# XuyangBai/D3Feat

Hardware: NVIDIA H100
Metric: points/sec through KPFCNN encoder (higher is better)
Workload: dtype f32

## Files before the change

### d3feat_b200/csrc/neighbors.cu

```cuda
#include <stdlib.h>

#include "ops.cuh"
#include "sort.cuh"

namespace d3f {

struct NbGrid {
  float minx, miny, minz, inv_cell;
  int nx, ny, nz;
  long long ncells;
};

static NbGrid make_grid(const float* host_bbox, float radius) {
  NbGrid g;
  float cell = radius * 1.001f;
  g.inv_cell = 1.0f / cell;
  g.minx = host_bbox[0];
  g.miny = host_bbox[1];
  g.minz = host_bbox[2];
  auto dim = [&](int a) {
    double ext = (double)host_bbox[3 + a] - (double)host_bbox[a];
    if (!(ext >= 0)) ext = 0;
    double n = floor(ext / (double)cell) + 2.0;
    return n > 2.0e9 ? 2000000000 : (int)n;
  };
  g.nx = dim(0);
  g.ny = dim(1);
  g.nz = dim(2);
  g.ncells = (long long)g.nx * g.ny * g.nz;
  return g;
}

constexpr long long kMaxGridCells = 1ll << 27;

__device__ __forceinline__ int cell_coord(float v, float mn, float inv, int n) {
  int c = (int)floorf((v - mn) * inv);
  return min(max(c, 0), n - 1);
}

__global__ void __launch_bounds__(256)
cell_count_kernel(const float* __restrict__ s, int Ns_cap, const int* __restrict__ ns_dev,
                  const int* __restrict__ start, int B, NbGrid g, uint32_t* __restrict__ cell_id,
                  int* __restrict__ cell_cnt) {
  const int Ns = dyn_rows(Ns_cap, ns_dev);
  int i = blockIdx.x * blockDim.x + threadIdx.x;
  if (i >= Ns) return;
  int b = batch_of(start, B, i);
  int cx = cell_coord(s[3 * (size_t)i], g.minx, g.inv_cell, g.nx);
  int cy = cell_coord(s[3 * (size_t)i + 1], g.miny, g.inv_cell, g.ny);
  int cz = cell_coord(s[3 * (size_t)i + 2], g.minz, g.inv_cell, g.nz);
  uint32_t c = (uint32_t)((long long)b * g.ncells + ((long long)cz * g.ny + cy) * g.nx + cx);
  cell_id[i] = c;
  atomicAdd(&cell_cnt[c], 1);
}

__global__ void __launch_bounds__(256)
cell_scatter_kernel(const float* __restrict__ s, int Ns_cap, const int* __restrict__ ns_dev,
                    const uint32_t* __restrict__ cell_id, const int* __restrict__ cell_start,
                    int* __restrict__ cell_cnt, float4* __restrict__ sorted_pts) {
  const int Ns = dyn_rows(Ns_cap, ns_dev);
  int i = blockIdx.x * blockDim.x + threadIdx.x;
  if (i >= Ns) return;
  uint32_t c = cell_id[i];
  int pos = cell_start[c] + atomicSub(&cell_cnt[c], 1) - 1;
  sorted_pts[pos] = make_float4(s[3 * (size_t)i], s[3 * (size_t)i + 1], s[3 * (size_t)i + 2], __uint_as_float((uint32_t)i));
}

__global__ void __launch_bounds__(256)
cell_order_kernel(const float4* __restrict__ sorted_pts, int Ns, int* __restrict__ out) {
  int i = blockIdx.x * blockDim.x + threadIdx.x;
  if (i < Ns) out[i] = (int)__float_as_uint(sorted_pts[i].w);
}

struct NbWs {
  uint32_t* cell_id;
  int* s_start;
  int* q_start;
  float4* sorted_pts;
  int* cell_start;
  int* cell_cnt;
  int* scan_scratch;
};

static size_t carve_nb(Carver& cv, int Ns, int B, long long total_cells, NbWs& w) {
  int n = Ns > 0 ? Ns : 1;
  w.cell_id = cv.take<uint32_t>(n);
  w.s_start = cv.take<int>(B + 1);
  w.q_start = cv.take<int>(B + 1);
  w.sorted_pts = cv.take<float4>(n);
  w.cell_start = cv.take<int>((size_t)total_cells + 1);
  w.cell_cnt = cv.take<int>((size_t)total_cells + 1);
  w.scan_scratch = cv.take<int>((size_t)scan_num_blocks((int)total_cells) + 1);
  return cv.off;
}

size_t radius_neighbors_workspace_bytes(int Ns, int B, float radius, const float* host_bbox) {
  if (host_bbox == nullptr || !(radius > 0.f) || B < 1) return 0;
  NbGrid g = make_grid(host_bbox, radius);
  long long total = g.ncells * B;
  if (total > kMaxGridCells) return 0;
  Carver cv(nullptr, ~(size_t)0);
  NbWs w;
  return carve_nb(cv, Ns, B, total, w) + 256;
}

int radius_neighbors_build(const float* supports, const int* s_batch_len, int B, int Ns, float radius,
                           const float* host_bbox, void* workspace, size_t workspace_bytes, cudaStream_t stream,
                           const int* ns_dev, const int* s_start_pre) {
  D3F_REQUIRE(B >= 1 && B <= kMaxBatch, D3F_ERR_INVALID, "radius_neighbors: B=%d must be in [1,%d]", B, kMaxBatch);
  D3F_REQUIRE(radius > 0.f && Ns >= 0 && host_bbox != nullptr, D3F_ERR_INVALID,
              "radius_neighbors: radius=%g Ns=%d invalid or host_bbox missing", (double)radius, Ns);
  NbGrid g = make_grid(host_bbox, radius);
  long long total = g.ncells * B;
  D3F_REQUIRE(total <= kMaxGridCells, D3F_ERR_CAPACITY,
              "radius_neighbors: grid %d x %d x %d x %d clouds exceeds %lld cells", g.nx, g.ny, g.nz, B,
              kMaxGridCells);
  D3F_REQUIRE(workspace_bytes >= radius_neighbors_workspace_bytes(Ns, B, radius, host_bbox), D3F_ERR_WORKSPACE,
              "radius_neighbors: workspace too small");
  Carver cv(workspace, workspace_bytes);
  NbWs w;
  carve_nb(cv, Ns, B, total, w);
  if (s_start_pre != nullptr) w.s_start = const_cast<int*>(s_start_pre);
  else if (launch_batch_start(s_batch_len, B, w.s_start, stream)) return D3F_ERR_CUDA;
  D3F_CUDA(cudaMemsetAsync(w.cell_cnt, 0, sizeof(int) * ((size_t)total + 1), stream));
  if (Ns == 0) {
    D3F_CUDA(cudaMemsetAsync(w.cell_start, 0, sizeof(int) * ((size_t)total + 1), stream));
    return D3F_OK;
  }
  cell_count_kernel<<<ceil_div(Ns, 256), 256, 0, stream>>>(supports, Ns, ns_dev, w.s_start, B, g, w.cell_id, w.cell_cnt);
  D3F_LAUNCH_CHECK("cell_count_kernel");
  if (exclusive_scan_i32(w.cell_cnt, w.cell_start, (int)total, w.cell_start + total, w.scan_scratch, stream))
    return D3F_ERR_CUDA;
  cell_scatter_kernel<<<ceil_div(Ns, 256), 256, 0, stream>>>(supports, Ns, ns_dev, w.cell_id, w.cell_start, w.cell_cnt,
                                                             w.sorted_pts);
  D3F_LAUNCH_CHECK("cell_scatter_kernel");
  return D3F_OK;
}

int radius_neighbors_order(const void* workspace, int Ns, int B, float radius, const float* host_bbox, int* out_order,
                           cudaStream_t stream) {
  D3F_REQUIRE(B >= 1 && radius > 0.f && host_bbox != nullptr, D3F_ERR_INVALID, "radius_neighbors_order: bad arguments");
  if (Ns <= 0) return D3F_OK;
  NbGrid g = make_grid(host_bbox, radius);
  long long total = g.ncells * B;
  D3F_REQUIRE(total <= kMaxGridCells, D3F_ERR_CAPACITY, "radius_neighbors: grid too large");
  Carver cv(const_cast<void*>(workspace), ~(size_t)0);
  NbWs w;
  carve_nb(cv, Ns, B, total, w);
  cell_order_kernel<<<ceil_div(Ns, 256), 256, 0, stream>>>(w.sorted_pts, Ns, out_order);
  D3F_LAUNCH_CHECK("cell_order_kernel");
  return D3F_OK;
}

constexpr int kNbWarps = 8;
constexpr int kNbListCap = 512;

struct Hit {
  float d2;
  int idx;
};

__device__ __forceinline__ bool hit_less(float da, int ia, float db, int ib) {
  return da < db || (da == db && ia < ib);
}

__device__ __forceinline__ float sq_dist_rn(float qx, float qy, float qz, float4 s) {
  float dx = __fsub_rn(qx, s.x), dy = __fsub_rn(qy, s.y), dz = __fsub_rn(qz, s.z);
  float r = __fmul_rn(dx, dx);
  r = __fadd_rn(r, __fmul_rn(dy, dy));
  r = __fadd_rn(r, __fmul_rn(dz, dz));
  return r;
}

template <int K>
__device__ __forceinline__ void bitonic_block2(unsigned& ka, unsigned& kb, int lane) {
  const bool asc = K == 64 || (lane & (K >> 1)) == 0;
#pragma unroll
  for (int j = K >> 1; j >= 2; j >>= 1) {
    const unsigned oa = __shfl_xor_sync(0xffffffffu, ka, j >> 1), ob = __shfl_xor_sync(0xffffffffu, kb, j >> 1);
    const bool keep_min = ((lane & (j >> 1)) == 0) == asc;
    ka = keep_min ? min(ka, oa) : max(ka, oa);
    kb = keep_min ? min(kb, ob) : max(kb, ob);
  }
  const unsigned lo = min(ka, kb), hi = max(ka, kb);
  ka = asc ? lo : hi;
  kb = asc ? hi : lo;
}

template <bool FILL>
__global__ void __launch_bounds__(kNbWarps * 32)
radius_query_kernel(const float* __restrict__ q, int Nq_cap, const int* __restrict__ nq_dev,
                    const int* __restrict__ q_start, int B, NbGrid g, const float4* __restrict__ sorted_pts,
                    const int* __restrict__ cell_start, float r2, int cols, int pad_value_in,
                    const int* __restrict__ pad_dev, int* __restrict__ counts, int* __restrict__ out_max,
                    int* __restrict__ out_idx) {
  const int Nq = dyn_rows(Nq_cap, nq_dev);
  const int pad_value = pad_dev ? __ldg(pad_dev) : pad_value_in;
  __shared__ int2 run_tab[kNbWarps][10];
  __shared__ Hit list[FILL ? kNbWarps : 1][FILL ? kNbListCap : 1];
  const int lane = threadIdx.x & 31, warp = threadIdx.x >> 5;
  const int qi = blockIdx.x * kNbWarps + warp;
  if (qi >= Nq) return;
  const float qx = q[3 * (size_t)qi], qy = q[3 * (size_t)qi + 1], qz = q[3 * (size_t)qi + 2];
  int b;
  if (B <= 32) {
    const bool le = lane < B && __ldg(q_start + lane) <= qi;
    b = max(__popc(__ballot_sync(0xffffffffu, le)) - 1, 0);
  } else {
    b = batch_of(q_start, B, qi);
  }
  const int cx = cell_coord(qx, g.minx, g.inv_cell, g.nx);
  const int cy = cell_coord(qy, g.miny, g.inv_cell, g.ny);
  const int cz = cell_coord(qz, g.minz, g.inv_cell, g.nz);

  int rs = 0, rl = 0;
  if (lane < 9) {
    const int dz = (lane * 11) >> 5;
    const int yy = cy + (lane - 3 * dz) - 1, zz = cz + dz - 1;
    if (yy >= 0 && yy < g.ny && zz >= 0 && zz < g.nz) {
      const int row = b * (int)g.ncells + (zz * g.ny + yy) * g.nx;
      const int x0 = max(cx - 1, 0), x1 = min(cx + 1, g.nx - 1);
      const int s = __ldg(cell_start + row + x0), e = __ldg(cell_start + row + x1 + 1);
      if (e > s) {
        rs = s;
        rl = e - s;
      }
    }
  }
  int inc = rl;
#pragma unroll
  for (int o = 1; o < 16; o <<= 1) {
    int t = __shfl_up_sync(0xffffffffu, inc, o);
    if (lane >= o) inc += t;
  }
  if (lane < 9) run_tab[warp][lane] = make_int2(inc, rs - (inc - rl));
  const int T = __shfl_sync(0xffffffffu, inc, 8);
  if (lane == 9) run_tab[warp][9] = make_int2(0x7fffffff, 0);
  __syncwarp();

  int n = 0;
  const int2* tp = &run_tab[warp][0];
  int2 cur = *tp;
  const unsigned below = (1u << lane) - 1u;
  for (int t0 = 0; t0 < T; t0 += 32) {
    const int t = t0 + lane;
    bool hit = false;
    float d2 = 0.f;
    int sidx = 0;
    if (t < T) {
      while (t >= cur.x) cur = *++tp;
      const float4 sp = __ldg(sorted_pts + (t + cur.y));
      d2 = sq_dist_rn(qx, qy, qz, sp);
      sidx = (int)__float_as_uint(sp.w);
      hit = d2 < r2;
    }
    const unsigned m = __ballot_sync(0xffffffffu, hit);
    if (FILL) {
      const int pos = n + __popc(m & below);
      if (hit && pos < kNbListCap) {
        list[warp][pos].d2 = d2;
        list[warp][pos].idx = sidx;
      }
    }
    n += __popc(m);
  }

  if (!FILL) {
    if (lane == 0) {
      counts[qi] = n;
      atomicMax(out_max, n);
    }
    return;
  }
  if (counts != nullptr && lane == 0) counts[qi] = n;
  if (out_max != nullptr && lane == 0) atomicMax(out_max, n);
  __syncwarp();
  int* row = out_idx + (size_t)qi * cols;
  bool sorted_fast = false;
  if (n <= 64) {
    const int ia = 2 * lane, ib = ia + 1;
    unsigned ka = 0xffffffffu, kb = 0xffffffffu;
    if (ia < n) ka = (__float_as_uint(list[warp][ia].d2) & ~63u) | (unsigned)ia;
    if (ib < n) kb = (__float_as_uint(list[warp][ib].d2) & ~63u) | (unsigned)ib;
    const int kmax = n <= 2 ? 2 : 2 << (31 - __clz(n - 1));
    if (kmax >= 2) bitonic_block2<2>(ka, kb, lane);
    if (kmax >= 4) bitonic_block2<4>(ka, kb, lane);
    if (kmax >= 8) bitonic_block2<8>(ka, kb, lane);
    if (kmax >= 16) bitonic_block2<16>(ka, kb, lane);
    if (kmax >= 32) bitonic_block2<32>(ka, kb, lane);
    if (kmax >= 64) bitonic_block2<64>(ka, kb, lane);
    const unsigned next_a = __shfl_down_sync(0xffffffffu, ka, 1);
    const bool clash = (ib < n && ((ka ^ kb) < 64u)) || (ib + 1 < n && lane < 31 && ((kb ^ next_a) < 64u));
    if (!__any_sync(0xffffffffu, clash)) {
      if (ia < n && ia < cols) row[ia] = list[warp][ka & 63u].idx;
      if (ib < n && ib < cols) row[ib] = list[warp][kb & 63u].idx;
      sorted_fast = true;
    }
  }
  if (sorted_fast) {
  } else if (n <= 64) {
    const unsigned long long kInf = ~0ull;
    unsigned long long a = kInf, b = kInf;
    if (lane < n) a = ((unsigned long long)__float_as_uint(list[warp][lane].d2) << 32) | (unsigned)list[warp][lane].idx;
    if (n <= 32) {
#pragma unroll
      for (int k = 2; k <= 32; k <<= 1) {
#pragma unroll
        for (int j = k >> 1; j > 0; j >>= 1) {
          unsigned long long o = __shfl_xor_sync(0xffffffffu, a, j);
          bool keep_min = ((lane & j) == 0) == ((lane & k) == 0);
          a = (keep_min == (o < a)) ? o : a;
        }
      }
      if (lane < n && lane < cols) row[lane] = (int)(unsigned)a;
    } else {
      if (lane + 32 < n)
        b = ((unsigned long long)__float_as_uint(list[warp][lane + 32].d2) << 32) | (unsigned)list[warp][lane + 32].idx;
#pragma unroll
      for (int k = 2; k <= 64; k <<= 1) {
#pragma unroll
        for (int j = k >> 1; j > 0; j >>= 1) {
          if (j == 32) {
            unsigned long long lo = a < b ? a : b, hi = a < b ? b : a;
            a = lo;
            b = hi;
          } else {
            unsigned long long oa = __shfl_xor_sync(0xffffffffu, a, j), ob = __shfl_xor_sync(0xffffffffu, b, j);
            bool lower = (lane & j) == 0;
            bool asc_a = (lane & k) == 0;
            bool asc_b = ((lane + 32) & k) == 0;
            a = ((lower == asc_a) == (oa < a)) ? oa : a;
            b = ((lower == asc_b) == (ob < b)) ? ob : b;
          }
        }
      }
      if (lane < cols) row[lane] = (int)(unsigned)a;
      if (lane + 32 < n && lane + 32 < cols) row[lane + 32] = (int)(unsigned)b;
    }
  } else if (n <= kNbListCap) {
    for (int j = lane; j < n; j += 32) {
      float dj = list[warp][j].d2;
      int ij = list[warp][j].idx;
      int rank = 0;
      for (int k = 0; k < n; ++k) rank += hit_less(list[warp][k].d2, list[warp][k].idx, dj, ij) ? 1 : 0;
      if (rank < cols) row[rank] = ij;
    }
  } else {
    float last_d = -1.f;
    int last_i = -1;
    int emit = min(n, cols);
    for (int c = 0; c < emit; ++c) {
      float best_d = 3.0e38f;
      int best_i = 0x7fffffff;
      for (int t = lane; t < T; t += 32) {
        int r = 0;
#pragma unroll
        for (int k = 0; k < 8; ++k) r += (t >= run_tab[warp][k].x) ? 1 : 0;
        float4 sp = sorted_pts[t + run_tab[warp][r].y];
        float d2 = sq_dist_rn(qx, qy, qz, sp);
        int si = (int)__float_as_uint(sp.w);
        if (d2 < r2 && hit_less(last_d, last_i, d2, si) && hit_less(d2, si, best_d, best_i)) {
          best_d = d2;
          best_i = si;
        }
      }
#pragma unroll
      for (int o = 16; o > 0; o >>= 1) {
        float od = __shfl_xor_sync(0xffffffffu, best_d, o);
        int oi = __shfl_xor_sync(0xffffffffu, best_i, o);
        if (hit_less(od, oi, best_d, best_i)) {
          best_d = od;
          best_i = oi;
        }
      }
      if (lane == 0) row[c] = best_i;
      last_d = best_d;
      last_i = best_i;
    }
  }
  for (int c = n + lane; c < cols; c += 32) row[c] = pad_value;
}

constexpr int kNbListCap2 = 256;

__device__ __forceinline__ void cex_dir(unsigned& a, unsigned& b, bool asc) {
  const unsigned lo = min(a, b), hi = max(a, b);
  a = asc ? lo : hi;
  b = asc ? hi : lo;
}
template <int K>
__device__ __forceinline__ void bitonic_block4(unsigned (&k)[4], int hl) {
  if (K == 2) {
    cex_dir(k[0], k[1], true);
    cex_dir(k[2], k[3], false);
    return;
  }
  const bool asc = K == 64 || (hl & (K >> 2)) == 0;
#pragma unroll
  for (int j = K >> 1; j >= 4; j >>= 1) {
    const bool keep_min = ((hl & (j >> 2)) == 0) == asc;
#pragma unroll
    for (int e = 0; e < 4; ++e) {
      const unsigned o = __shfl_xor_sync(0xffffffffu, k[e], j >> 2);
      k[e] = keep_min ? min(k[e], o) : max(k[e], o);
    }
  }
  cex_dir(k[0], k[2], asc);
  cex_dir(k[1], k[3], asc);
  cex_dir(k[0], k[1], asc);
  cex_dir(k[2], k[3], asc);
}

__global__ void __launch_bounds__(kNbWarps * 32, 6)
radius_query2_kernel(const float* __restrict__ q, int Nq_cap, const int* __restrict__ nq_dev,
                     const int* __restrict__ q_start, int B, NbGrid g, const float4* __restrict__ sorted_pts,
                     const int* __restrict__ cell_start, float r2, int cols, int pad_value_in,
                     const int* __restrict__ pad_dev, int* __restrict__ counts, int* __restrict__ out_max,
                     int* __restrict__ out_idx) {
  const int Nq = dyn_rows(Nq_cap, nq_dev);
  const int pad_value = pad_dev ? __ldg(pad_dev) : pad_value_in;
  __shared__ int2 run_tab[kNbWarps * 2][10];
  __shared__ Hit list[kNbWarps * 2][kNbListCap2];
  const int lane = threadIdx.x & 31, warp = threadIdx.x >> 5;
  const int hw = lane >> 4, hl = lane & 15;
  const int slot = warp * 2 + hw;
  const int qi_raw = (blockIdx.x * kNbWarps + warp) * 2 + hw;
  if ((blockIdx.x * kNbWarps + warp) * 2 >= Nq) return;
  const bool qvalid = qi_raw < Nq;
  const int qi = qvalid ? qi_raw : Nq - 1;
  const unsigned hmask = 0xffffu << (16 * hw);
  const float qx = q[3 * (size_t)qi], qy = q[3 * (size_t)qi + 1], qz = q[3 * (size_t)qi + 2];
  int b;
  if (B <= 16) {
    const bool le = hl < B && __ldg(q_start + hl) <= qi;
    b = max(__popc((__ballot_sync(0xffffffffu, le) >> (16 * hw)) & 0xffffu) - 1, 0);
  } else {
    b = batch_of(q_start, B, qi);
  }
  const int cx = cell_coord(qx, g.minx, g.inv_cell, g.nx);
  const int cy = cell_coord(qy, g.miny, g.inv_cell, g.ny);
  const int cz = cell_coord(qz, g.minz, g.inv_cell, g.nz);
  int rs = 0, rl = 0;
  if (hl < 9) {
    const int dz = (hl * 11) >> 5;
    const int yy = cy + (hl - 3 * dz) - 1, zz = cz + dz - 1;
    if (yy >= 0 && yy < g.ny && zz >= 0 && zz < g.nz) {
      const int row = b * (int)g.ncells + (zz * g.ny + yy) * g.nx;
      const int x0 = max(cx - 1, 0), x1 = min(cx + 1, g.nx - 1);
      const int s = __ldg(cell_start + row + x0), e = __ldg(cell_start + row + x1 + 1);
      if (e > s) {
        rs = s;
        rl = e - s;
      }
    }
  }
  int inc = rl;
#pragma unroll
  for (int o = 1; o < 16; o <<= 1) {
    const int t = __shfl_up_sync(0xffffffffu, inc, o, 16);
    if (hl >= o) inc += t;
  }
  if (hl < 9) run_tab[slot][hl] = make_int2(inc, rs - (inc - rl));
  int T = __shfl_sync(0xffffffffu, inc, 8, 16);
  if (!qvalid) T = 0;
  if (hl == 9) run_tab[slot][9] = make_int2(0x7fffffff, 0);
  __syncwarp();
  const int Tmax = max(T, __shfl_xor_sync(0xffffffffu, T, 16));

  int n = 0;
  const int2* tp = &run_tab[slot][0];
  int2 cur = *tp;
  const unsigned below = (1u << hl) - 1u;
  for (int t0 = 0; t0 < Tmax; t0 += 16) {
    const int t = t0 + hl;
    bool hit = false;
    float d2 = 0.f;
    int sidx = 0;
    if (t < T) {
      while (t >= cur.x) cur = *++tp;
      const float4 sp = __ldg(sorted_pts + (t + cur.y));
      d2 = sq_dist_rn(qx, qy, qz, sp);
      sidx = (int)__float_as_uint(sp.w);
      hit = d2 < r2;
    }
    const unsigned m = (__ballot_sync(0xffffffffu, hit) >> (16 * hw)) & 0xffffu;
    const int pos = n + __popc(m & below);
    if (hit && pos < kNbListCap2) {
      list[slot][pos].d2 = d2;
      list[slot][pos].idx = sidx;
    }
    n += __popc(m);
  }
  if (qvalid && hl == 0) {
    if (counts != nullptr) counts[qi] = n;
    if (out_max != nullptr) atomicMax(out_max, n);
  }
  __syncwarp();
  int* row = out_idx + (size_t)qi * cols;

  bool done = !qvalid;
  {
    const int nmax = max(n, __shfl_xor_sync(0xffffffffu, n, 16));
    const bool mine = qvalid && n <= 64;
    unsigned k[4];
#pragma unroll
    for (int e = 0; e < 4; ++e) {
      const int i = 4 * hl + e;
      k[e] = (mine && i < n) ? ((__float_as_uint(list[slot][i].d2) & ~63u) | (unsigned)i) : 0xffffffffu;
    }
    const int nsort = min(nmax, 64);
    const int kmax = nsort <= 2 ? 2 : 2 << (31 - __clz(nsort - 1));
    if (kmax >= 2) bitonic_block4<2>(k, hl);
    if (kmax >= 4) bitonic_block4<4>(k, hl);
    if (kmax >= 8) bitonic_block4<8>(k, hl);
    if (kmax >= 16) bitonic_block4<16>(k, hl);
    if (kmax >= 32) bitonic_block4<32>(k, hl);
    if (kmax >= 64) bitonic_block4<64>(k, hl);
    const unsigned next0 = __shfl_down_sync(0xffffffffu, k[0], 1, 16);
    const int i0 = 4 * hl;
    bool clash = (i0 + 1 < n && ((k[0] ^ k[1]) < 64u)) || (i0 + 2 < n && ((k[1] ^ k[2]) < 64u)) ||
                 (i0 + 3 < n && ((k[2] ^ k[3]) < 64u)) || (i0 + 4 < n && hl < 15 && ((k[3] ^ next0) < 64u));
    const bool any_clash = ((__ballot_sync(0xffffffffu, mine && clash) >> (16 * hw)) & 0xffffu) != 0u;
    if (mine && !any_clash) {
#pragma unroll
      for (int e = 0; e < 4; ++e) {
        const int i = i0 + e;
        if (i < n && i < cols) row[i] = list[slot][k[e] & 63u].idx;
      }
      done = true;
    }
  }
  if (!done) {
    if (n <= kNbListCap2) {
      for (int j = hl; j < n; j += 16) {
        const float dj = list[slot][j].d2;
        const int ij = list[slot][j].idx;
        int rank = 0;
        for (int kk = 0; kk < n; ++kk) rank += hit_less(list[slot][kk].d2, list[slot][kk].idx, dj, ij) ? 1 : 0;
        if (rank < cols) row[rank] = ij;
      }
    } else {
      float last_d = -1.f;
      int last_i = -1;
      const int emit = min(n, cols);
      for (int c = 0; c < emit; ++c) {
        float best_d = 3.0e38f;
        int best_i = 0x7fffffff;
        for (int t = hl; t < T; t += 16) {
          int r = 0;
#pragma unroll
          for (int kk = 0; kk < 8; ++kk) r += (t >= run_tab[slot][kk].x) ? 1 : 0;
          const float4 sp = sorted_pts[t + run_tab[slot][r].y];
          const float d2 = sq_dist_rn(qx, qy, qz, sp);
          const int si = (int)__float_as_uint(sp.w);
          if (d2 < r2 && hit_less(last_d, last_i, d2, si) && hit_less(d2, si, best_d, best_i)) {
            best_d = d2;
            best_i = si;
          }
        }
#pragma unroll
        for (int o = 8; o > 0; o >>= 1) {
          const float od = __shfl_xor_sync(hmask, best_d, o);
          const int oi = __shfl_xor_sync(hmask, best_i, o);
          if (hit_less(od, oi, best_d, best_i)) {
            best_d = od;
            best_i = oi;
          }
        }
        if (hl == 0) row[c] = best_i;
        last_d = best_d;
        last_i = best_i;
      }
    }
  }
  if (qvalid)
    for (int c = n + hl; c < cols; c += 16) row[c] = pad_value;
}

static int query_common(bool fill, const float* queries, const int* q_batch_len, int Nq, int B, int Ns, float radius,
                        const float* host_bbox, const void* workspace, int cols, int pad_value, int* counts,
                        int* out_max, int* out_idx, cudaStream_t stream, const int* nq_dev = nullptr,
                        const int* pad_dev = nullptr, const int* q_start_pre = nullptr) {
  D3F_REQUIRE(B >= 1 && B <= kMaxBatch && Nq >= 0 && radius > 0.f && host_bbox != nullptr, D3F_ERR_INVALID,
              "radius_neighbors: invalid arguments (B=%d Nq=%d radius=%g)", B, Nq, (double)radius);
  NbGrid g = make_grid(host_bbox, radius);
  long long total = g.ncells * B;
  D3F_REQUIRE(total <= kMaxGridCells, D3F_ERR_CAPACITY, "radius_neighbors: grid too large");
  Carver cv(const_cast<void*>(workspace), ~(size_t)0);
  NbWs w;
  carve_nb(cv, Ns, B, total, w);
  if (q_start_pre != nullptr) w.q_start = const_cast<int*>(q_start_pre);
  else if (launch_batch_start(q_batch_len, B, w.q_start, stream)) return D3F_ERR_CUDA;
  if (out_max != nullptr && !fill) D3F_CUDA(cudaMemsetAsync(out_max, 0, sizeof(int), stream));
  if (Nq == 0) return D3F_OK;
  float r2 = radius * radius;
  int blocks = ceil_div(Nq, kNbWarps);
  const char* hv = getenv("D3F_NB_HALFWARP");
  if (fill && !(hv != nullptr && hv[0] == '0')) {
    radius_query2_kernel<<<ceil_div(Nq, kNbWarps * 2), kNbWarps * 32, 0, stream>>>(
        queries, Nq, nq_dev, w.q_start, B, g, w.sorted_pts, w.cell_start, r2, cols, pad_value, pad_dev, counts, out_max,
        out_idx);
    D3F_LAUNCH_CHECK("radius_query2_kernel");
    return D3F_OK;
  }
  if (fill) {
    radius_query_kernel<true><<<blocks, kNbWarps * 32, 0, stream>>>(queries, Nq, nq_dev, w.q_start, B, g, w.sorted_pts,
                                                                    w.cell_start, r2, cols, pad_value, pad_dev,
                                                                    counts, out_max, out_idx);
  } else {
    radius_query_kernel<false><<<blocks, kNbWarps * 32, 0, stream>>>(queries, Nq, nq_dev, w.q_start, B, g, w.sorted_pts,
                                                                     w.cell_start, r2, 0, 0, nullptr, counts,
                                                                     out_max, nullptr);
  }
  D3F_LAUNCH_CHECK("radius_query_kernel");
  return D3F_OK;
}

int radius_neighbors_count(const float* queries, const int* q_batch_len, int Nq, int B, int Ns, float radius,
                           const float* host_bbox, const void* workspace, int* counts, int* out_max,
                           cudaStream_t stream) {
  D3F_REQUIRE(counts != nullptr && out_max != nullptr, D3F_ERR_INVALID, "radius_neighbors_count: null output");
  return query_common(false, queries, q_batch_len, Nq, B, Ns, radius, host_bbox, workspace, 0, 0, counts, out_max,
                      nullptr, stream);
}

int radius_neighbors_fill(const float* queries, const int* q_batch_len, int Nq, int B, int Ns, float radius,
                          const float* host_bbox, const void* workspace, int cols, int pad_value, int* out_idx,
                          cudaStream_t stream, const int* nq_dev, const int* pad_dev, const int* q_start_pre) {
  D3F_REQUIRE(cols >= 0 && (out_idx != nullptr || cols == 0 || Nq == 0), D3F_ERR_INVALID,
              "radius_neighbors_fill: cols=%d / null output", cols);
  if (cols == 0) return D3F_OK;
  return query_common(true, queries, q_batch_len, Nq, B, Ns, radius, host_bbox, workspace, cols, pad_value, nullptr,
                      nullptr, out_idx, stream, nq_dev, pad_dev, q_start_pre);
}

}
```

### d3feat_b200/csrc/ops.cuh

```cuda
#pragma once
#include "common.cuh"

namespace d3f {

struct Epilogue {
  const float* rowscale;
  const float* bn_scale;
  const float* bn_shift;
  const float* bias;
  const float* residual;
  float leaky_alpha;
  const int* row_map;
  const int* m_dev = nullptr;
  int m_off = 0;
};
int gemm_f32(const float* A, const float* B, float* C, int M, int N, int K, const Epilogue& ep, cudaStream_t stream);

size_t tc_packed_floats(int K, int N);
int tc_padded_n(int N);
int tc_pack_weight(const float* W, int K, int N, float* packed, cudaStream_t stream);
bool tc_gemm_supported(const float* A, int K);
int tc_gemm(const float* A, const float* Bp, float* C, int M, int N, int K, const Epilogue& ep, cudaStream_t stream,
            float* split_ws = nullptr, const float* A2 = nullptr, int K1 = 0);
int tc_gemm_splits(int M, int N, int K);
size_t tc_gemm_split_ws_floats(int M, int N, int K);

int launch_batch_start(const int* len, int B, int* start, cudaStream_t stream);
int bbox_device(const float* pts, int N, float* out_bbox, cudaStream_t stream);
size_t grid_subsample_workspace_bytes(int N, int B);
int grid_subsample(const float* pts, const int* batch_len, int B, int N, float dl, const float* feats, int fdim,
                   const int* classes, int ldim, const float* host_bbox, float* out_pts, float* out_feats,
                   int* out_classes, int* out_batch_len, int* out_M, void* workspace, size_t workspace_bytes,
                   cudaStream_t stream, const int* n_dev = nullptr, int out_capacity = -1, int* status = nullptr,
                   const int* start_pre = nullptr);

size_t radius_neighbors_workspace_bytes(int Ns, int B, float radius, const float* host_bbox);
int radius_neighbors_build(const float* supports, const int* s_batch_len, int B, int Ns, float radius,
                           const float* host_bbox, void* workspace, size_t workspace_bytes, cudaStream_t stream,
                           const int* ns_dev = nullptr, const int* s_start_pre = nullptr);
int radius_neighbors_count(const float* queries, const int* q_batch_len, int Nq, int B, int Ns, float radius,
                           const float* host_bbox, const void* workspace, int* counts, int* out_max,
                           cudaStream_t stream);
int radius_neighbors_order(const void* workspace, int Ns, int B, float radius, const float* host_bbox, int* out_order,
                           cudaStream_t stream);
int radius_neighbors_fill(const float* queries, const int* q_batch_len, int Nq, int B, int Ns, float radius,
                          const float* host_bbox, const void* workspace, int cols, int pad_value, int* out_idx,
                          cudaStream_t stream, const int* nq_dev = nullptr, const int* pad_dev = nullptr,
                          const int* q_start_pre = nullptr);

size_t pyramid_workspace_bytes(int B, const d3f_pyramid_spec* spec, const int* capacity, const float* host_bbox);
int pyramid_build(const float* points, const int* lengths, int B, int N0, const d3f_pyramid_spec* spec,
                  const float* host_bbox, float* const* out_points, int* const* out_lengths,
                  int* const* out_neighbors, int* const* out_pools, int* const* out_upsamples, const int* capacity,
                  int* out_level_sizes, void* workspace, size_t workspace_bytes, cudaStream_t stream,
                  int* d_counts = nullptr, int* d_status = nullptr, const int* n0_dev = nullptr);

size_t kpconv_workspace_bytes(int Nq, int Ns, int H, int K, int Cin, int Cout);
int kpconv_forward_impl(bool deform, const float* q, const float* s, const int* idx, const float* feat,
                        const float* Kp, const float* offsets, const float* modulations, const float* W,
                        const float* W_packed, const int* query_order, int Nq,
                        int Ns, int H, int K, int Cin, int Cout, float extent, int influence, int mode, int normalize,
                        const float* bn_scale, const float* bn_shift, const float* bias, float leaky_alpha,
                        float* out, void* workspace, size_t workspace_bytes, cudaStream_t stream,
                        const int* nq_dev = nullptr, const int* ns_dev = nullptr);

bool kpconv_fused_supported(int Nq, int H, int K, int Cin, int Cout, int influence, int mode, const float* feat,
                            const float* W, const float* out, const int* query_order);
size_t kpconv_fused_workspace_bytes();
int kpconv_fused_forward(const float* q, const float4* s4, const int* idx, const float* feat, const float* Kp,
                         const float* W, float* w_img, int Nq, int Ns, int H, int Cout, float extent, int normalize,
                         const float* bn_scale, const float* bn_shift, const float* bias, float leaky_alpha, float* out,
                         cudaStream_t stream, const int* nq_dev = nullptr, const int* ns_dev = nullptr);

int ind_max_pool(const float* x, const int* inds, int N1, int N2, int H, int C, float* out, void* workspace,
                 size_t workspace_bytes, cudaStream_t stream, const int* n1_dev = nullptr, const int* n2_dev = nullptr);
int closest_pool(const float* x, const int* inds, int N1, int N2, int ld_inds, int C, float* out,
                 cudaStream_t stream, const int* n1_dev = nullptr, const int* n2_dev = nullptr);
int l2_normalize(const float* x, int N, int C, float eps, float* out, cudaStream_t stream, const int* n_dev = nullptr);
size_t detection_scores_workspace_bytes(int N, int B);
int detection_scores(const float* feats, const int* neighbors, const int* lengths, int B, int N, int H, int D,
                     float* out_scores, void* workspace, size_t workspace_bytes, cudaStream_t stream,
                     const int* n_dev = nullptr);
int affine_leaky(const float* x, int N, int C, const float* scale, const float* shift, const float* residual,
                 float alpha, float* out, cudaStream_t stream, const int* n_dev = nullptr);

size_t select_keypoints_workspace_bytes(int N, int B);
int select_keypoints(const float* scores, const int* lengths, int B, int N, int k, const float* points,
                     const float* descriptors, int D, int* out_order, int* out_index, int* out_count, float* out_points,
                     float* out_descriptors, float* out_scores, void* workspace, size_t workspace_bytes,
                     cudaStream_t stream, const int* n_dev = nullptr);

}
```

### d3feat_b200/csrc/pyramid.cu

```cuda
#include <math.h>

#include "ops.cuh"

namespace d3f {

namespace {

struct GridSlot {
  int level;
  float radius;
  void* ws;
  size_t bytes;
};

struct PyramidPlan {
  int L;
  const d3f_pyramid_spec* spec;
};

inline bool same_radius(float a, float b) { return fabsf(a - b) <= 1e-6f * fmaxf(fabsf(a), fabsf(b)); }

}

size_t pyramid_workspace_bytes(int B, const d3f_pyramid_spec* spec, const int* capacity, const float* host_bbox) {
  if (spec == nullptr || capacity == nullptr || host_bbox == nullptr) return 0;
  int L = spec->n_levels;
  if (L < 1 || L > D3F_MAX_LEVELS) return 0;
  size_t total = align_up(grid_subsample_workspace_bytes(capacity[0], B) + 512, 256);
  total += align_up(sizeof(int) * (size_t)D3F_MAX_LEVELS * (B + 1), 256);
  for (int l = 0; l < L; ++l) {
    float radii[3] = {spec->conv_radius[l], spec->sub_dl[l] > 0.f ? spec->pool_radius[l] : -1.f,
                      (l > 0 && spec->sub_dl[l - 1] > 0.f) ? spec->up_radius[l - 1] : -1.f};
    for (int a = 0; a < 3; ++a) {
      if (!(radii[a] > 0.f)) continue;
      bool dup = false;
      for (int b = 0; b < a; ++b) dup = dup || (radii[b] > 0.f && same_radius(radii[a], radii[b]));
      if (dup) continue;
      size_t nb = radius_neighbors_workspace_bytes(capacity[l], B, radii[a], host_bbox);
      if (nb == 0) return 0;
      total += align_up(nb, 256);
    }
  }
  return total + 1024;
}

__global__ void set_count_kernel(int* __restrict__ dst, int value, const int* __restrict__ src) {
  *dst = src ? *src : value;
}

int pyramid_build(const float* points, const int* lengths, int B, int N0, const d3f_pyramid_spec* spec,
                  const float* host_bbox, float* const* out_points, int* const* out_lengths,
                  int* const* out_neighbors, int* const* out_pools, int* const* out_upsamples, const int* capacity,
                  int* out_level_sizes, void* workspace, size_t workspace_bytes, cudaStream_t stream, int* d_counts,
                  int* d_status, const int* n0_dev) {
  D3F_REQUIRE(spec != nullptr && capacity != nullptr && host_bbox != nullptr, D3F_ERR_INVALID,
              "pyramid_build: null argument");
  const bool exact = out_level_sizes != nullptr;
  D3F_REQUIRE(exact || (d_counts != nullptr && d_status != nullptr), D3F_ERR_INVALID,
              "pyramid_build: the static form needs d_counts and d_status");
  const int L = spec->n_levels;
  D3F_REQUIRE(L >= 1 && L <= D3F_MAX_LEVELS, D3F_ERR_INVALID, "pyramid_build: n_levels=%d", L);
  D3F_REQUIRE(N0 >= 0 && N0 <= capacity[0], D3F_ERR_CAPACITY, "pyramid_build: N0=%d exceeds capacity %d", N0, capacity[0]);
  D3F_REQUIRE(workspace_bytes >= pyramid_workspace_bytes(B, spec, capacity, host_bbox) &&
                  pyramid_workspace_bytes(B, spec, capacity, host_bbox) > 0,
              D3F_ERR_WORKSPACE, "pyramid_build: workspace too small (or grid too large)");

  char* base = (char*)workspace;
  size_t off = 0;
  void* sub_ws = base;
  size_t sub_bytes = align_up(grid_subsample_workspace_bytes(capacity[0], B) + 512, 256);
  off += sub_bytes;
  int* starts = (int*)(base + off);
  off += align_up(sizeof(int) * (size_t)D3F_MAX_LEVELS * (B + 1), 256);
  if (launch_batch_start(lengths, B, starts, stream)) return D3F_ERR_CUDA;
  int* counts = d_counts != nullptr ? d_counts : (int*)((char*)sub_ws + sub_bytes - 256);
  int* status = d_status != nullptr ? d_status : counts + D3F_MAX_LEVELS;
  if (d_status == nullptr) D3F_CUDA(cudaMemsetAsync(status, 0, sizeof(int), stream));
  set_count_kernel<<<1, 1, 0, stream>>>(counts, N0, n0_dev);
  D3F_LAUNCH_CHECK("set_count_kernel");

  GridSlot slots[3 * D3F_MAX_LEVELS];
  int n_slots = 0;
  const float* lvl_pts[D3F_MAX_LEVELS];
  const int* lvl_len[D3F_MAX_LEVELS];
  int lvl_n[D3F_MAX_LEVELS];
  lvl_pts[0] = points;
  lvl_len[0] = lengths;
  lvl_n[0] = exact ? N0 : capacity[0];

  auto grid_for = [&](int l, float radius, GridSlot** out) -> int {
    for (int i = 0; i < n_slots; ++i)
      if (slots[i].level == l && same_radius(slots[i].radius, radius)) {
        *out = &slots[i];
        return D3F_OK;
      }
    GridSlot& g = slots[n_slots];
    g.level = l;
    g.radius = radius;
    g.bytes = align_up(radius_neighbors_workspace_bytes(capacity[l], B, radius, host_bbox), 256);
    g.ws = base + off;
    off += g.bytes;
    D3F_REQUIRE(off <= workspace_bytes, D3F_ERR_WORKSPACE, "pyramid_build: workspace exhausted");
    int rc = radius_neighbors_build(lvl_pts[l], lvl_len[l], B, lvl_n[l], radius, host_bbox, g.ws, g.bytes, stream,
                                    counts + l, starts + (size_t)l * (B + 1));
    if (rc) return rc;
    ++n_slots;
    *out = &g;
    return D3F_OK;
  };
  auto fill = [&](int lq, int ls, GridSlot* g, int lim, int* out) -> int {
    return radius_neighbors_fill(lvl_pts[lq], lvl_len[lq], lvl_n[lq], B, lvl_n[ls], g->radius, host_bbox, g->ws, lim,
                                 lvl_n[ls], out, stream, counts + lq, counts + ls, starts + (size_t)lq * (B + 1));
  };

  for (int l = 0; l < L; ++l) {
    const int lim = spec->limit[l];
    D3F_REQUIRE(lim >= 1, D3F_ERR_INVALID, "pyramid_build: limit[%d]=%d", l, lim);
    if (exact) out_level_sizes[l] = lvl_n[l];
    GridSlot* g = nullptr;
    if (spec->conv_radius[l] > 0.f) {
      int rc = grid_for(l, spec->conv_radius[l], &g);
      if (rc) return rc;
      rc = fill(l, l, g, lim, out_neighbors[l]);
      if (rc) return rc;
    }
    if (spec->sub_dl[l] > 0.f && l + 1 < L) {
      D3F_REQUIRE(out_points[l + 1] != nullptr && out_lengths[l + 1] != nullptr, D3F_ERR_INVALID,
                  "pyramid_build: missing output buffers for level %d", l + 1);
      int* d_M = counts + l + 1;
      int rc = grid_subsample(lvl_pts[l], lvl_len[l], B, lvl_n[l], spec->sub_dl[l], nullptr, 0, nullptr, 0, host_bbox,
                              out_points[l + 1], nullptr, nullptr, out_lengths[l + 1], d_M, sub_ws, sub_bytes - 256,
                              stream, counts + l, capacity[l + 1], status, starts + (size_t)l * (B + 1));
      if (rc) return rc;
      if (launch_batch_start(out_lengths[l + 1], B, starts + (size_t)(l + 1) * (B + 1), stream)) return D3F_ERR_CUDA;
      int M = capacity[l + 1];
      if (exact) {
        D3F_CUDA(cudaMemcpyAsync(&M, d_M, sizeof(int), cudaMemcpyDeviceToHost, stream));
        D3F_CUDA(cudaStreamSynchronize(stream));
        D3F_REQUIRE(M != -1, D3F_ERR_CAPACITY, "pyramid_build: points fall outside the supplied bbox at level %d", l);
        D3F_REQUIRE(M >= 0, D3F_ERR_CAPACITY, "pyramid_build: level %d exceeds its capacity %d", l + 1, capacity[l + 1]);
      }
      lvl_pts[l + 1] = out_points[l + 1];
      lvl_len[l + 1] = out_lengths[l + 1];
      lvl_n[l + 1] = M;
      rc = grid_for(l, spec->pool_radius[l], &g);
      if (rc) return rc;
      rc = fill(l + 1, l, g, lim, out_pools[l]);
      if (rc) return rc;
      rc = grid_for(l + 1, spec->up_radius[l], &g);
      if (rc) return rc;
      rc = fill(l, l + 1, g, lim, out_upsamples[l]);
      if (rc) return rc;
    } else if (l + 1 < L) {
      D3F_REQUIRE(false, D3F_ERR_INVALID, "pyramid_build: level %d has no subsampling but is not the last level", l);
    }
  }
  return D3F_OK;
}

}
```

Baseline: 61.36 million.

## Process radius queries in cell-sorted order and share candidate scans between paired queries

Neighbor fill queries now iterate in the grid's cell-sorted point order, reusing the sorted float4 buffer and the precomputed cell ids. Cell coordinates are decoded with fast multiply-shift division instead of being recomputed from the coordinates. When the two half-warp queries in a warp touch identical cell runs, the full warp scans the candidates once and tests both queries, which avoids redundant loads and gives better lane utilization. This adds divergence checks and extra shuffles, and it relies on the sorted points being spatially coherent.

```diff
diff --git a/d3feat_b200/csrc/neighbors.cu b/d3feat_b200/csrc/neighbors.cu
--- a/d3feat_b200/csrc/neighbors.cu
+++ b/d3feat_b200/csrc/neighbors.cu
@@ -4,11 +4,32 @@
 #include "sort.cuh"
 
 namespace d3f {
+
+constexpr long long kMaxGridCells = 1ll << 27;
+
+struct FastDiv {
+  unsigned m;
+  int s;
+};
+
+static FastDiv make_fast_div(long long d) {
+  FastDiv f{0u, 0};
+  if (d < 2 || d > kMaxGridCells) return f;
+  int lg = 0;
+  while ((1ll << lg) < d) ++lg;
+  const int k = lg + 27 > 32 ? lg + 27 : 32;
+  f.m = (unsigned)((1ull << k) / (unsigned long long)d + 1ull);
+  f.s = k - 32;
+  return f;
+}
+
+__device__ __forceinline__ unsigned fast_div(unsigned n, FastDiv f) { return __umulhi(n, f.m) >> f.s; }
 
 struct NbGrid {
   float minx, miny, minz, inv_cell;
   int nx, ny, nz;
   long long ncells;
+  FastDiv div_x, div_y, div_cells;
 };
 
 static NbGrid make_grid(const float* host_bbox, float radius) {
@@ -28,10 +49,11 @@
   g.ny = dim(1);
   g.nz = dim(2);
   g.ncells = (long long)g.nx * g.ny * g.nz;
+  g.div_x = make_fast_div(g.nx);
+  g.div_y = make_fast_div(g.ny);
+  g.div_cells = make_fast_div(g.ncells);
   return g;
 }
-
-constexpr long long kMaxGridCells = 1ll << 27;
 
 __device__ __forceinline__ int cell_coord(float v, float mn, float inv, int n) {
   int c = (int)floorf((v - mn) * inv);
@@ -149,6 +171,21 @@
   carve_nb(cv, Ns, B, total, w);
   cell_order_kernel<<<ceil_div(Ns, 256), 256, 0, stream>>>(w.sorted_pts, Ns, out_order);
   D3F_LAUNCH_CHECK("cell_order_kernel");
+  return D3F_OK;
+}
+
+int radius_neighbors_cell_order(const void* workspace, int Ns, int B, float radius, const float* host_bbox,
+                                const float4** sorted_pts, const uint32_t** cell_id) {
+  D3F_REQUIRE(workspace != nullptr && B >= 1 && radius > 0.f && host_bbox != nullptr, D3F_ERR_INVALID,
+              "radius_neighbors_cell_order: bad arguments");
+  NbGrid g = make_grid(host_bbox, radius);
+  long long total = g.ncells * B;
+  D3F_REQUIRE(total <= kMaxGridCells, D3F_ERR_CAPACITY, "radius_neighbors: grid too large");
+  Carver cv(const_cast<void*>(workspace), ~(size_t)0);
+  NbWs w;
+  carve_nb(cv, Ns, B, total, w);
+  *sorted_pts = w.sorted_pts;
+  *cell_id = w.cell_id;
   return D3F_OK;
 }
 
@@ -416,7 +453,8 @@
                      const int* __restrict__ q_start, int B, NbGrid g, const float4* __restrict__ sorted_pts,
                      const int* __restrict__ cell_start, float r2, int cols, int pad_value_in,
                      const int* __restrict__ pad_dev, int* __restrict__ counts, int* __restrict__ out_max,
-                     int* __restrict__ out_idx) {
+                     int* __restrict__ out_idx, const float4* __restrict__ q_sorted,
+                     const uint32_t* __restrict__ q_cell) {
   const int Nq = dyn_rows(Nq_cap, nq_dev);
   const int pad_value = pad_dev ? __ldg(pad_dev) : pad_value_in;
   __shared__ int2 run_tab[kNbWarps * 2][10];
@@ -424,22 +462,47 @@
   const int lane = threadIdx.x & 31, warp = threadIdx.x >> 5;
   const int hw = lane >> 4, hl = lane & 15;
   const int slot = warp * 2 + hw;
-  const int qi_raw = (blockIdx.x * kNbWarps + warp) * 2 + hw;
+  const int qs_raw = (blockIdx.x * kNbWarps + warp) * 2 + hw;
   if ((blockIdx.x * kNbWarps + warp) * 2 >= Nq) return;
-  const bool qvalid = qi_raw < Nq;
-  const int qi = qvalid ? qi_raw : Nq - 1;
+  const bool qvalid = qs_raw < Nq;
+  const int qs = qvalid ? qs_raw : Nq - 1;
   const unsigned hmask = 0xffffu << (16 * hw);
-  const float qx = q[3 * (size_t)qi], qy = q[3 * (size_t)qi + 1], qz = q[3 * (size_t)qi + 2];
-  int b;
-  if (B <= 16) {
-    const bool le = hl < B && __ldg(q_start + hl) <= qi;
-    b = max(__popc((__ballot_sync(0xffffffffu, le) >> (16 * hw)) & 0xffffu) - 1, 0);
+  int qi;
+  float qx, qy, qz;
+  if (q_sorted != nullptr) {
+    const float4 p = __ldg(q_sorted + qs);
+    qx = p.x;
+    qy = p.y;
+    qz = p.z;
+    qi = (int)__float_as_uint(p.w);
   } else {
-    b = batch_of(q_start, B, qi);
-  }
-  const int cx = cell_coord(qx, g.minx, g.inv_cell, g.nx);
-  const int cy = cell_coord(qy, g.miny, g.inv_cell, g.ny);
-  const int cz = cell_coord(qz, g.minz, g.inv_cell, g.nz);
+    qi = qs;
+    qx = q[3 * (size_t)qi];
+    qy = q[3 * (size_t)qi + 1];
+    qz = q[3 * (size_t)qi + 2];
+  }
+  int b, cx, cy, cz;
+  if (q_cell != nullptr) {
+    const unsigned c = __ldg(q_cell + qi);
+    const unsigned bq = fast_div(c, g.div_cells);
+    const unsigned r = c - bq * (unsigned)g.ncells;
+    const unsigned yz = fast_div(r, g.div_x);
+    const unsigned zq = fast_div(yz, g.div_y);
+    b = (int)bq;
+    cx = (int)(r - yz * (unsigned)g.nx);
+    cy = (int)(yz - zq * (unsigned)g.ny);
+    cz = (int)zq;
+  } else {
+    if (B <= 16) {
+      const bool le = hl < B && __ldg(q_start + hl) <= qi;
+      b = max(__popc((__ballot_sync(0xffffffffu, le) >> (16 * hw)) & 0xffffu) - 1, 0);
+    } else {
+      b = batch_of(q_start, B, qi);
+    }
+    cx = cell_coord(qx, g.minx, g.inv_cell, g.nx);
+    cy = cell_coord(qy, g.miny, g.inv_cell, g.ny);
+    cz = cell_coord(qz, g.minz, g.inv_cell, g.nz);
+  }
   int rs = 0, rl = 0;
   if (hl < 9) {
     const int dz = (hl * 11) >> 5;
@@ -466,12 +529,52 @@
   if (hl == 9) run_tab[slot][9] = make_int2(0x7fffffff, 0);
   __syncwarp();
   const int Tmax = max(T, __shfl_xor_sync(0xffffffffu, T, 16));
+  const int rs_other = __shfl_xor_sync(0xffffffffu, rs, 16), rl_other = __shfl_xor_sync(0xffffffffu, rl, 16);
+  const bool same_runs = __ballot_sync(0xffffffffu, !qvalid || rs != rs_other || rl != rl_other) == 0u;
 
   int n = 0;
+  if (same_runs) {
+    const float ax = __shfl_sync(0xffffffffu, qx, 0), ay = __shfl_sync(0xffffffffu, qy, 0),
+                az = __shfl_sync(0xffffffffu, qz, 0);
+    const float bx = __shfl_sync(0xffffffffu, qx, 16), by = __shfl_sync(0xffffffffu, qy, 16),
+                bz = __shfl_sync(0xffffffffu, qz, 16);
+    const int2* tp = &run_tab[warp * 2][0];
+    int2 cur = *tp;
+    const unsigned below = (1u << lane) - 1u;
+    int na = 0, nb = 0;
+    for (int t0 = 0; t0 < T; t0 += 32) {
+      const int t = t0 + lane;
+      bool ha = false, hb = false;
+      float da = 0.f, db = 0.f;
+      int sidx = 0;
+      if (t < T) {
+        while (t >= cur.x) cur = *++tp;
+        const float4 sp = __ldg(sorted_pts + (t + cur.y));
+        da = sq_dist_rn(ax, ay, az, sp);
+        db = sq_dist_rn(bx, by, bz, sp);
+        sidx = (int)__float_as_uint(sp.w);
+        ha = da < r2;
+        hb = db < r2;
+      }
+      const unsigned ma = __ballot_sync(0xffffffffu, ha), mb = __ballot_sync(0xffffffffu, hb);
+      const int pa = na + __popc(ma & below), pb = nb + __popc(mb & below);
+      if (ha && pa < kNbListCap2) {
+        list[warp * 2][pa].d2 = da;
+        list[warp * 2][pa].idx = sidx;
+      }
+      if (hb && pb < kNbListCap2) {
+        list[warp * 2 + 1][pb].d2 = db;
+        list[warp * 2 + 1][pb].idx = sidx;
+      }
+      na += __popc(ma);
+      nb += __popc(mb);
+    }
+    n = hw ? nb : na;
+  }
   const int2* tp = &run_tab[slot][0];
   int2 cur = *tp;
   const unsigned below = (1u << hl) - 1u;
-  for (int t0 = 0; t0 < Tmax; t0 += 16) {
+  for (int t0 = 0; t0 < (same_runs ? 0 : Tmax); t0 += 16) {
     const int t = t0 + hl;
     bool hit = false;
     float d2 = 0.f;
@@ -580,7 +683,8 @@
 static int query_common(bool fill, const float* queries, const int* q_batch_len, int Nq, int B, int Ns, float radius,
                         const float* host_bbox, const void* workspace, int cols, int pad_value, int* counts,
                         int* out_max, int* out_idx, cudaStream_t stream, const int* nq_dev = nullptr,
-                        const int* pad_dev = nullptr, const int* q_start_pre = nullptr) {
+                        const int* pad_dev = nullptr, const int* q_start_pre = nullptr,
+                        const float4* q_sorted = nullptr, const uint32_t* q_cell = nullptr) {
   D3F_REQUIRE(B >= 1 && B <= kMaxBatch && Nq >= 0 && radius > 0.f && host_bbox != nullptr, D3F_ERR_INVALID,
               "radius_neighbors: invalid arguments (B=%d Nq=%d radius=%g)", B, Nq, (double)radius);
   NbGrid g = make_grid(host_bbox, radius);
@@ -599,7 +703,7 @@
   if (fill && !(hv != nullptr && hv[0] == '0')) {
     radius_query2_kernel<<<ceil_div(Nq, kNbWarps * 2), kNbWarps * 32, 0, stream>>>(
         queries, Nq, nq_dev, w.q_start, B, g, w.sorted_pts, w.cell_start, r2, cols, pad_value, pad_dev, counts, out_max,
-        out_idx);
+        out_idx, q_sorted, q_cell);
     D3F_LAUNCH_CHECK("radius_query2_kernel");
     return D3F_OK;
   }
@@ -626,12 +730,14 @@
 
 int radius_neighbors_fill(const float* queries, const int* q_batch_len, int Nq, int B, int Ns, float radius,
                           const float* host_bbox, const void* workspace, int cols, int pad_value, int* out_idx,
-                          cudaStream_t stream, const int* nq_dev, const int* pad_dev, const int* q_start_pre) {
+                          cudaStream_t stream, const int* nq_dev, const int* pad_dev, const int* q_start_pre,
+                          const float4* q_sorted, const uint32_t* q_cell) {
   D3F_REQUIRE(cols >= 0 && (out_idx != nullptr || cols == 0 || Nq == 0), D3F_ERR_INVALID,
               "radius_neighbors_fill: cols=%d / null output", cols);
+  D3F_REQUIRE(q_cell == nullptr || q_sorted != nullptr, D3F_ERR_INVALID, "radius_neighbors_fill: q_cell without q_sorted");
   if (cols == 0) return D3F_OK;
   return query_common(true, queries, q_batch_len, Nq, B, Ns, radius, host_bbox, workspace, cols, pad_value, nullptr,
-                      nullptr, out_idx, stream, nq_dev, pad_dev, q_start_pre);
-}
-
-}
+                      nullptr, out_idx, stream, nq_dev, pad_dev, q_start_pre, q_sorted, q_cell);
+}
+
+}
diff --git a/d3feat_b200/csrc/ops.cuh b/d3feat_b200/csrc/ops.cuh
--- a/d3feat_b200/csrc/ops.cuh
+++ b/d3feat_b200/csrc/ops.cuh
@@ -43,10 +43,13 @@
                            cudaStream_t stream);
 int radius_neighbors_order(const void* workspace, int Ns, int B, float radius, const float* host_bbox, int* out_order,
                            cudaStream_t stream);
+int radius_neighbors_cell_order(const void* workspace, int Ns, int B, float radius, const float* host_bbox,
+                                const float4** sorted_pts, const uint32_t** cell_id);
 int radius_neighbors_fill(const float* queries, const int* q_batch_len, int Nq, int B, int Ns, float radius,
                           const float* host_bbox, const void* workspace, int cols, int pad_value, int* out_idx,
                           cudaStream_t stream, const int* nq_dev = nullptr, const int* pad_dev = nullptr,
-                          const int* q_start_pre = nullptr);
+                          const int* q_start_pre = nullptr, const float4* q_sorted = nullptr,
+                          const uint32_t* q_cell = nullptr);
 
 size_t pyramid_workspace_bytes(int B, const d3f_pyramid_spec* spec, const int* capacity, const float* host_bbox);
 int pyramid_build(const float* points, const int* lengths, int B, int N0, const d3f_pyramid_spec* spec,
diff --git a/d3feat_b200/csrc/pyramid.cu b/d3feat_b200/csrc/pyramid.cu
--- a/d3feat_b200/csrc/pyramid.cu
+++ b/d3feat_b200/csrc/pyramid.cu
@@ -108,9 +108,19 @@
     *out = &g;
     return D3F_OK;
   };
-  auto fill = [&](int lq, int ls, GridSlot* g, int lim, int* out) -> int {
+  auto fill = [&](int lq, int ls, GridSlot* g, int lim, int* out, const float4* q_sorted,
+                  const uint32_t* q_cell) -> int {
     return radius_neighbors_fill(lvl_pts[lq], lvl_len[lq], lvl_n[lq], B, lvl_n[ls], g->radius, host_bbox, g->ws, lim,
-                                 lvl_n[ls], out, stream, counts + lq, counts + ls, starts + (size_t)lq * (B + 1));
+                                 lvl_n[ls], out, stream, counts + lq, counts + ls, starts + (size_t)lq * (B + 1),
+                                 q_sorted, q_cell);
+  };
+  auto cell_order = [&](int l, GridSlot* g, const float4** sorted, const uint32_t** cell) -> int {
+    *sorted = nullptr;
+    *cell = nullptr;
+    for (int i = 0; i < n_slots && g == nullptr; ++i)
+      if (slots[i].level == l) g = &slots[i];
+    if (g == nullptr) return D3F_OK;
+    return radius_neighbors_cell_order(g->ws, lvl_n[l], B, g->radius, host_bbox, sorted, cell);
   };
 
   for (int l = 0; l < L; ++l) {
@@ -121,7 +131,11 @@
     if (spec->conv_radius[l] > 0.f) {
       int rc = grid_for(l, spec->conv_radius[l], &g);
       if (rc) return rc;
-      rc = fill(l, l, g, lim, out_neighbors[l]);
+      const float4* q_sorted;
+      const uint32_t* q_cell;
+      rc = cell_order(l, g, &q_sorted, &q_cell);
+      if (rc) return rc;
+      rc = fill(l, l, g, lim, out_neighbors[l], q_sorted, q_cell);
       if (rc) return rc;
     }
     if (spec->sub_dl[l] > 0.f && l + 1 < L) {
@@ -145,11 +159,15 @@
       lvl_n[l + 1] = M;
       rc = grid_for(l, spec->pool_radius[l], &g);
       if (rc) return rc;
-      rc = fill(l + 1, l, g, lim, out_pools[l]);
+      rc = fill(l + 1, l, g, lim, out_pools[l], nullptr, nullptr);
       if (rc) return rc;
       rc = grid_for(l + 1, spec->up_radius[l], &g);
       if (rc) return rc;
-      rc = fill(l, l + 1, g, lim, out_upsamples[l]);
+      const float4* q_sorted;
+      const uint32_t* q_cell;
+      rc = cell_order(l, nullptr, &q_sorted, &q_cell);
+      if (rc) return rc;
+      rc = fill(l, l + 1, g, lim, out_upsamples[l], q_sorted, nullptr);
       if (rc) return rc;
     } else if (l + 1 < L) {
       D3F_REQUIRE(false, D3F_ERR_INVALID, "pyramid_build: level %d has no subsampling but is not the last level", l);
```

Result: no change. 61.86 million (median of 6 runs) (+0.8%).
